# mosure/bevy_gaussian_splatting

Hardware: NVIDIA H100
Metric: rendered Msplats/sec @1080p, 6M-gaussian cloud (higher is better)
Workload: dtype f32 (f16-packed inputs)

## Files before the change

### bevy_gaussian_splatting_b200/csrc/project.cu

```cuda
#include <cuda_fp16.h>

#include "project_math.cuh"

namespace bgs {

__constant__ float c_shc[16] = {
    0.28209479177387814f, -0.4886025119029199f, 0.4886025119029199f, -0.4886025119029199f,
    1.0925484305920792f, -1.0925484305920792f, 0.31539156525252005f, -1.0925484305920792f,
    0.5462742152960396f, -0.5900435899266435f, 2.890611442640554f, -0.4570457994644658f,
    0.3731763325901154f, -0.4570457994644658f, 1.445305721320277f, -0.5900435899266435f};

__device__ __forceinline__ void normalize3(const float a[3], float out[3]) {
    const float inv = rsqrtf((a[0] * a[0] + a[1] * a[1]) + a[2] * a[2]);
    out[0] = a[0] * inv; out[1] = a[1] * inv; out[2] = a[2] * inv;
}
__device__ __forceinline__ float dot3(const float a[3], const float b[3]) {
    return (a[0] * b[0] + a[1] * b[1]) + a[2] * b[2];
}
__device__ __forceinline__ float srgb_to_linear(float v) {
    if (v <= 0.04045f) return v * (1.0f / 12.92f);
    return __powf((v + 0.055f) * (1.0f / 1.055f), 2.4f);
}
__device__ __forceinline__ uint32_t pack_bbox(float lo, float hi) {
    return (uint32_t)(int)lo | ((uint32_t)(int)hi << 16);
}
constexpr uint32_t BBOX_EMPTY = 1u;

__device__ __forceinline__ void make_bbox(float cx, float cy, float hx, float hy, int Wi, int Hi,
                                          uint32_t& bx, uint32_t& by) {
    bx = BBOX_EMPTY; by = BBOX_EMPTY;
    if (!(hx >= 0.0f) || !(hy >= 0.0f) || !(cx == cx) || !(cy == cy)) return;
    const float sx = hx * 1.0e-3f + 1.0e-2f, sy = hy * 1.0e-3f + 1.0e-2f;
    float x0 = ceilf((cx - hx) - (0.5f + sx));
    float x1 = floorf((cx + hx) - (0.5f - sx));
    float y0 = ceilf((cy - hy) - (0.5f + sy));
    float y1 = floorf((cy + hy) - (0.5f - sy));
    if (!(x0 <= x1) || !(y0 <= y1)) return;
    x0 = fmaxf(x0, 0.0f); y0 = fmaxf(y0, 0.0f);
    x1 = fminf(x1, (float)(Wi - 1)); y1 = fminf(y1, (float)(Hi - 1));
    if (!(x0 <= x1) || !(y0 <= y1)) return;
    bx = pack_bbox(x0, x1); by = pack_bbox(y0, y1);
}

template <bool F16>
struct Attr;
template <>
struct Attr<false> {
    __device__ static float4 load(const void* blocks, uint32_t id, float* sh, float q[4], float so[4], bool need_sh,
                                  uint32_t* = nullptr) {
        const float4* b = reinterpret_cast<const float4*>(blocks) + (size_t)id * 16;
        const float4 p = __ldg(b), r = __ldg(b + 1), s = __ldg(b + 2);
        q[0] = r.x; q[1] = r.y; q[2] = r.z; q[3] = r.w;
        so[0] = s.x; so[1] = s.y; so[2] = s.z; so[3] = s.w;
        if (need_sh) {
#pragma unroll
            for (int i = 0; i < 12; ++i) {
                const float4 v = __ldg(b + 3 + i);
                sh[4 * i] = v.x; sh[4 * i + 1] = v.y; sh[4 * i + 2] = v.z; sh[4 * i + 3] = v.w;
            }
        }
        return p;
    }
};
template <>
struct Attr<true> {
    __device__ static float lo(uint32_t w) { return __half2float(__ushort_as_half((unsigned short)(w & 0xFFFFu))); }
    __device__ static float hi(uint32_t w) { return __half2float(__ushort_as_half((unsigned short)(w >> 16))); }
    __device__ static float4 load(const void* blocks, uint32_t id, float* sh, float q[4], float so[4], bool need_sh,
                                  uint32_t* op_bits = nullptr) {
        const uint4* b = reinterpret_cast<const uint4*>(blocks) + (size_t)id * 8;
        const uint4 pw = __ldg(b), w = __ldg(b + 1);
        if (op_bits) *op_bits = w.w & 0xFFFFu;
        q[0] = hi(w.x); q[1] = lo(w.x); q[2] = hi(w.y); q[3] = lo(w.y);
        so[0] = hi(w.z); so[1] = lo(w.z); so[2] = hi(w.w); so[3] = lo(w.w);
        if (need_sh) {
#pragma unroll
            for (int i = 0; i < 6; ++i) {
                const uint4 v = __ldg(b + 2 + i);
                sh[8 * i] = lo(v.x); sh[8 * i + 1] = hi(v.x); sh[8 * i + 2] = lo(v.y); sh[8 * i + 3] = hi(v.y);
                sh[8 * i + 4] = lo(v.z); sh[8 * i + 5] = hi(v.z); sh[8 * i + 6] = lo(v.w); sh[8 * i + 7] = hi(v.w);
            }
        }
        return make_float4(__uint_as_float(pw.x), __uint_as_float(pw.y), __uint_as_float(pw.z), __uint_as_float(pw.w));
    }
};

template <bool F16>
__global__ void repack_kernel(const uint4* __restrict__ pos, const uint4* __restrict__ sh, const uint4* __restrict__ rot,
                              const uint4* __restrict__ so, uint32_t n, uint4* __restrict__ blocks) {
    constexpr uint32_t CH = F16 ? 8u : 16u;
    constexpr uint32_t SHC = F16 ? 6u : 12u;
    const size_t i = (size_t)blockIdx.x * blockDim.x + threadIdx.x;
    if (i >= (size_t)n * CH) return;
    const uint32_t id = (uint32_t)(i / CH), c = (uint32_t)(i % CH);
    uint4 v = make_uint4(0u, 0u, 0u, 0u);
    if (c == 0) v = pos[id];
    else if (c == 1) v = rot[id];
    else if (!F16 && c == 2) v = so[id];
    else {
        const uint32_t k = c - (F16 ? 2u : 3u);
        if (k < SHC) v = sh[(size_t)id * SHC + k];
    }
    blocks[i] = v;
}
void launch_repack(bool f16, const void* pos, const void* sh, const void* rot, const void* so, uint32_t n, void* blocks,
                   cudaStream_t stream) {
    const size_t total = (size_t)n * (f16 ? 8 : 16);
    const uint32_t grid = (uint32_t)((total + 255) / 256);
    if (f16) repack_kernel<true><<<grid, 256, 0, stream>>>((const uint4*)pos, (const uint4*)sh, (const uint4*)rot, (const uint4*)so, n, (uint4*)blocks);
    else repack_kernel<false><<<grid, 256, 0, stream>>>((const uint4*)pos, (const uint4*)sh, (const uint4*)rot, (const uint4*)so, n, (uint4*)blocks);
}

__global__ void depth_range_kernel(const float4* __restrict__ pos, uint32_t n, const uint32_t* __restrict__ sorted_payload,
                                   const uint32_t* __restrict__ slot_ids ,
                                   FrameCounters* __restrict__ ctr, FrameConsts fc) {
    if (threadIdx.x != 0 || blockIdx.x != 0 || n < 2u) return;
    const uint32_t n_vis = ctr->n_vis, n_sorted = ctr->n_sort;
    auto id_at = [&](uint32_t i) { const uint32_t p = sorted_payload[i]; return slot_ids ? slot_ids[p] : p; };
    uint32_t first, last;
    if (n_sorted == n) {
        first = id_at(1u); last = id_at(n - 1u);
    } else {
        const uint32_t cmin = 0xFFFFFFFFu - ctr->culled_min_inv, cmax = ctr->culled_max_p1 - 1u;
        first = n_vis >= 2u ? id_at(1u) : cmin;
        last = (n - n_vis) >= 1u ? cmax : id_at(n - 1u);
    }
    auto dist = [&](uint32_t id) {
        const float4 p = pos[id];
        float pw[4];
        mat4_point(fc.model, p.x, p.y, p.z, pw);
        const float d[3] = {pw[0] - fc.cam[0], pw[1] - fc.cam[1], pw[2] - fc.cam[2]};
        return sqrtf(dot3(d, d));
    };
    ctr->depth_min = dist(last);
    ctr->depth_max = dist(first);
}

__device__ __forceinline__ float adaptive_cutoff(float opacity) {
    const float a = 9.0f + 2.0f * det_ln(opacity);
    return sqrtf(a > 0.000001f ? a : 0.000001f);
}
__global__ void cutoff_table_kernel(float* __restrict__ tab) {
    const uint32_t h = blockIdx.x * blockDim.x + threadIdx.x;
    if (h < 65536u) tab[h] = adaptive_cutoff(__half2float(__ushort_as_half((unsigned short)h)));
}
void launch_cutoff_table(float* tab, cudaStream_t stream) { cutoff_table_kernel<<<256, 256, 0, stream>>>(tab); }

template <class ShLoader>
__device__ __forceinline__ void project_one(const FrameConsts& fc, const FrameCounters* __restrict__ ctr, uint32_t r, float4 p4,
                                            const float q[4], const float so[4], float cutoff_pre, ShLoader load_sh,
                                            SplatRec* __restrict__ recs, float4* __restrict__ extra, float4* __restrict__ aux) {
    SplatRec rec;
    rec.ux = 0.f; rec.uy = 0.f; rec.vx = 0.f; rec.vy = 0.f;
    rec.bx = BBOX_EMPTY; rec.by = BBOX_EMPTY;
    rec.r = 0.f; rec.g = 0.f; rec.b = 0.f;

    const KeyOut k = key_of(fc, p4.x, p4.y, p4.z);
    const float W = fc.W, H = fc.H;
    const float hw = 0.5f * W, hh = 0.5f * H;
    const float cx = k.ndc[0] * hw + hw;
    const float cy = hh - k.ndc[1] * hh;
    rec.cx = cx; rec.cy = cy;
    const float opacity = so[3];
    rec.op = opacity * fc.global_opacity;
    const bool drawn = k.visible && !(fc.draw_mode == BGS_DRAW_SELECTED && p4.w < 0.5f);

    float A[3][3];
#pragma unroll
    for (int rr = 0; rr < 3; ++rr)
#pragma unroll
        for (int cc = 0; cc < 3; ++cc) A[rr][cc] = fc.model[cc * 4 + rr];
    float Rm[3][3];
    {
        const float qr = q[0], x = q[1], y = q[2], z = q[3];
        Rm[0][0] = 1.0f - 2.0f * (y * y + z * z);
        Rm[1][0] = 2.0f * (x * y - qr * z);
        Rm[2][0] = 2.0f * (x * z + qr * y);
        Rm[0][1] = 2.0f * (x * y + qr * z);
        Rm[1][1] = 1.0f - 2.0f * (x * x + z * z);
        Rm[2][1] = 2.0f * (y * z - qr * x);
        Rm[0][2] = 2.0f * (x * z - qr * y);
        Rm[1][2] = 2.0f * (y * z + qr * x);
        Rm[2][2] = 1.0f - 2.0f * (x * x + y * y);
    }
    const float sc[3] = {so[0] * fc.global_scale, so[1] * fc.global_scale, so[2] * fc.global_scale};

    if (drawn) {
        float cutoff = 3.0f;
        if (fc.adaptive) {
            cutoff = cutoff_pre == cutoff_pre ? cutoff_pre : adaptive_cutoff(opacity);
        }
        if (fc.gaussian_mode == BGS_GAUSSIAN_3D) {
        float M[3][3], Sg[3][3], X[3][3], TS[3][3];
#pragma unroll
        for (int i = 0; i < 3; ++i)
#pragma unroll
            for (int j = 0; j < 3; ++j) M[i][j] = sc[i] * Rm[i][j];
#pragma unroll
        for (int i = 0; i < 3; ++i)
#pragma unroll
            for (int j = 0; j < 3; ++j) Sg[i][j] = (M[0][i] * M[0][j] + M[1][i] * M[1][j]) + M[2][i] * M[2][j];
        const float mn = fminf(fminf(fminf(fabsf(Sg[0][0]), fabsf(Sg[0][1])), fminf(fabsf(Sg[0][2]), fabsf(Sg[1][1]))),
                               fminf(fabsf(Sg[1][2]), fabsf(Sg[2][2])));
        const float mx = fmaxf(fmaxf(fmaxf(fabsf(Sg[0][0]), fabsf(Sg[0][1])), fmaxf(fabsf(Sg[0][2]), fabsf(Sg[1][1]))),
                               fmaxf(fabsf(Sg[1][2]), fabsf(Sg[2][2])));
        if (fc.model_identity && mn > 0.0f && mx < __uint_as_float(0x7F800000u) && Sg[0][0] == Sg[0][0] &&
            Sg[0][1] == Sg[0][1] && Sg[0][2] == Sg[0][2] && Sg[1][1] == Sg[1][1] && Sg[1][2] == Sg[1][2] && Sg[2][2] == Sg[2][2]) {
#pragma unroll
            for (int i = 0; i < 3; ++i)
#pragma unroll
                for (int j = 0; j < 3; ++j) TS[i][j] = Sg[i][j];
        } else {
#pragma unroll
        for (int i = 0; i < 3; ++i)
#pragma unroll
            for (int j = 0; j < 3; ++j) X[i][j] = (A[i][0] * Sg[0][j] + A[i][1] * Sg[1][j]) + A[i][2] * Sg[2][j];
#pragma unroll
        for (int i = 0; i < 3; ++i)
#pragma unroll
            for (int j = 0; j < 3; ++j) TS[i][j] = (X[i][0] * A[j][0] + X[i][1] * A[j][1]) + X[i][2] * A[j][2];
        }
        float c3[6] = {TS[0][0], TS[1][0], TS[2][0], TS[1][1], TS[2][1], TS[2][2]};
        if (fc.cov_pre) {
            c3[0] = q[0]; c3[1] = q[1]; c3[2] = q[2]; c3[3] = q[3]; c3[4] = so[0]; c3[5] = so[1];
        }
        const float Vrk[3][3] = {{c3[0], c3[1], c3[2]}, {c3[1], c3[3], c3[4]}, {c3[2], c3[4], c3[5]}};
        float tv[4];
        mat4_point(fc.view_from_world, k.pw[0], k.pw[1], k.pw[2], tv);
        const float fx = fc.p00 * W, fy = fc.p11 * H;
        const float sz = 1.0f / (tv[2] * tv[2]);
        const float J00 = fx / tv[2], J20 = -(fx * tv[0]) * sz;
        const float J11 = -fy / tv[2], J21 = (fy * tv[1]) * sz;
        float Tm[3][2];
#pragma unroll
        for (int i = 0; i < 3; ++i) {
            const float v0 = fc.view_from_world[i * 4 + 0], v1 = fc.view_from_world[i * 4 + 1],
                        v2 = fc.view_from_world[i * 4 + 2];
            Tm[i][0] = v0 * J00 + v2 * J20;
            Tm[i][1] = v1 * J11 + v2 * J21;
        }
        float Y[3][2];
#pragma unroll
        for (int i = 0; i < 3; ++i)
#pragma unroll
            for (int b = 0; b < 2; ++b) Y[i][b] = (Vrk[i][0] * Tm[0][b] + Vrk[i][1] * Tm[1][b]) + Vrk[i][2] * Tm[2][b];
        const float a = ((Tm[0][0] * Y[0][0] + Tm[1][0] * Y[1][0]) + Tm[2][0] * Y[2][0]) + 0.3f;
        const float b = (Tm[0][1] * Y[0][0] + Tm[1][1] * Y[1][0]) + Tm[2][1] * Y[2][0];
        const float c = ((Tm[0][1] * Y[0][1] + Tm[1][1] * Y[1][1]) + Tm[2][1] * Y[2][1]) + 0.3f;
        const float det = a * c - b * b;
        const float mid = 0.5f * (a + c);
        const float disc = fmaxf(0.0f, mid * mid - det);
        const float term = sqrtf(disc);
        const float l1 = mid + term;
        if (fc.aabb) {
            const float l2 = fmaxf(mid - term, 0.0f);
            const float Rq = cutoff * fmaxf(sqrtf(l1), sqrtf(l2));
            const float dinv = 1.0f / det;
            rec.ux = c * dinv; rec.uy = -b * dinv; rec.vx = a * dinv; rec.vy = Rq;
            const float h = 0.5f * Rq;
            make_bbox(cx, cy, h, h, fc.Wi, fc.Hi, rec.bx, rec.by);
        } else {
        const float aa = (a - c) * (a - c);
        const float bb = sqrtf(aa + (4.0f * b) * b);
        const float major = sqrtf(((a + c) + bb) * 0.5f);
        const float minor = sqrtf(((a + c) - bb) * 0.5f);
        const float Bx = cutoff * major, By = cutoff * minor;
        const float evx = -b, evy = l1 - a;
        const float el = sqrtf(evx * evx + evy * evy);
        const float e1x = evx / el, e1y = evy / el;
        const float e2x = e1y, e2y = -e1x;
        rec.ux = (2.0f * e1x) / Bx; rec.uy = (-2.0f * e1y) / Bx;
        rec.vx = (2.0f * e2x) / By; rec.vy = (-2.0f * e2y) / By;
        const float hx = 0.5f * (fabsf(e1x) * Bx + fabsf(e2x) * By);
        const float hy = 0.5f * (fabsf(e1y) * Bx + fabsf(e2y) * By);
        if (rec.ux == rec.ux && rec.uy == rec.uy && rec.vx == rec.vx && rec.vy == rec.vy)
            make_bbox(cx, cy, hx, hy, fc.Wi, fc.Hi, rec.bx, rec.by);
        }
        } else {
            float L[3][2];
#pragma unroll
            for (int j = 0; j < 2; ++j) {
                const float rc[3] = {Rm[j][0] * sc[j], Rm[j][1] * sc[j], Rm[j][2] * sc[j]};
#pragma unroll
                for (int i = 0; i < 3; ++i) L[i][j] = (A[i][0] * rc[0] + A[i][1] * rc[1]) + A[i][2] * rc[2];
            }
            float G[3][4];
            mat4_dir(fc.clip_from_world, L[0][0], L[1][0], L[2][0], G[0]);
            mat4_dir(fc.clip_from_world, L[0][1], L[1][1], L[2][1], G[1]);
            mat4_point(fc.clip_from_world, k.pw[0], k.pw[1], k.pw[2], G[2]);
            const float fxk = fc.p00 * W / 2.0f, fyk = fc.p11 * H / 2.0f;
            const float cxk = (W - 1.0f) / 2.0f, cyk = (H - 1.0f) / 2.0f;
            float T0[3], T1[3], T2[3];
#pragma unroll
            for (int j = 0; j < 3; ++j) {
                T0[j] = fxk * G[j][0] + cxk * G[j][3];
                T1[j] = fyk * G[j][1] + cyk * G[j][3];
                T2[j] = G[j][3];
            }
            const float c2 = cutoff * cutoff;
            const float test[3] = {c2, c2, -1.0f};
            const float tt[3] = {test[0] * T2[0], test[1] * T2[1], test[2] * T2[2]};
            const float d = dot3(tt, T2);
            float Rq = 0.0f, mean0 = 0.0f, mean1 = 0.0f;
            bool ok = !(fabsf(d) < 1.0e-4f);
            if (ok) {
                const float inv = 1.0f / d;
                const float f[3] = {inv * test[0], inv * test[1], inv * test[2]};
                const float t02[3] = {T0[0] * T2[0], T0[1] * T2[1], T0[2] * T2[2]};
                const float t12[3] = {T1[0] * T2[0], T1[1] * T2[1], T1[2] * T2[2]};
                mean0 = dot3(f, t02); mean1 = dot3(f, t12);
                const float f0[3] = {f[0] * T0[0], f[1] * T0[1], f[2] * T0[2]};
                const float f1[3] = {f[0] * T1[0], f[1] * T1[1], f[2] * T1[2]};
                const float ex = mean0 * mean0 - dot3(f0, T0);
                const float ey = mean1 * mean1 - dot3(f1, T1);
                if (ex < 1.0e-4f || ey < 1.0e-4f) ok = false;
                else Rq = fmaxf(fmaxf(sqrtf(ex), sqrtf(ey)), cutoff * 0.707106f);
            }
            if (ok) {
                rec.ux = 2.0f / Rq; rec.uy = 0.0f; rec.vx = 0.0f; rec.vy = -2.0f / Rq;
                const float h = 0.5f * Rq;
                if (Rq == Rq) make_bbox(cx, cy, h, h, fc.Wi, fc.Hi, rec.bx, rec.by);
                if (fc.aabb && extra != nullptr) {
                    float4* e = extra + (size_t)r * 4;
                    e[0] = make_float4(Rq, mean0, mean1, W / H);
                    e[1] = make_float4(T0[0], T0[1], T0[2], 0.0f);
                    e[2] = make_float4(T1[0], T1[1], T1[2], 0.0f);
                    e[3] = make_float4(T2[0], T2[1], T2[2], 0.0f);
                }
            }
        }

        float rgb[3] = {0.f, 0.f, 0.f};
        if (fc.rasterize_mode == BGS_RASTERIZE_COLOR) {
            float sh[48];
            load_sh(sh);
            const float dlt[3] = {k.pw[0] - fc.cam[0], k.pw[1] - fc.cam[1], k.pw[2] - fc.cam[2]};
            float dw[3], loc[3], dl[3];
            normalize3(dlt, dw);
            if (fc.model_identity) {
                loc[0] = dw[0]; loc[1] = dw[1]; loc[2] = dw[2];
            } else {
#pragma unroll
                for (int cc = 0; cc < 3; ++cc) {
                    const float col[3] = {A[0][cc], A[1][cc], A[2][cc]};
                    float bn[3];
                    normalize3(col, bn);
                    loc[cc] = dot3(bn, dw);
                }
            }
            normalize3(loc, dl);
            const float x = dl[0], y = dl[1], z = dl[2];
            const float xx = x * x, yy = y * y, zz = z * z;
            float basis[16];
            basis[0] = 1.0f;
            basis[1] = y; basis[2] = z; basis[3] = x;
            basis[4] = x * y; basis[5] = y * z; basis[6] = (2.0f * zz - xx) - yy;
            basis[7] = x * z; basis[8] = xx - yy;
            basis[9] = y * (3.0f * xx - yy);
            basis[10] = (x * y) * z;
            basis[11] = y * ((4.0f * zz - xx) - yy);
            basis[12] = z * ((2.0f * zz - 3.0f * xx) - 3.0f * yy);
            basis[13] = x * ((4.0f * zz - xx) - yy);
            basis[14] = z * (xx - yy);
            basis[15] = x * (xx - 3.0f * yy);
#pragma unroll
            for (int kk = 0; kk < 16; ++kk) basis[kk] *= c_shc[kk];
#pragma unroll
            for (int cc = 0; cc < 3; ++cc) {
                float acc = 0.5f;
#pragma unroll
                for (int kk = 0; kk < 16; ++kk) acc = fmaf(sh[3 * kk + cc], basis[kk], acc);
                rgb[cc] = acc;
            }
            if (fc.color_space == 0u) {
#pragma unroll
                for (int cc = 0; cc < 3; ++cc) rgb[cc] = srgb_to_linear(rgb[cc]);
            }
        }
        float drgb[3] = {0.f, 0.f, 0.f}, nrgb[3] = {0.f, 0.f, 0.f};
        if (fc.rasterize_mode == BGS_RASTERIZE_DEPTH || fc.aux) {
            float* rgb = drgb;
            const float dlt[3] = {k.pw[0] - fc.cam[0], k.pw[1] - fc.cam[1], k.pw[2] - fc.cam[2]};
            const float depth = sqrtf(dot3(dlt, dlt));
            const float dmin = ctr->depth_min, dmax = ctr->depth_max;
            if (fc.n_cloud >= 2u) {
            float nd = (depth - dmin) / (dmax - dmin);
            nd = fminf(fmaxf(nd, 0.0f), 1.0f);
            float t1 = (nd - 0.5f) / (1.0f - 0.5f); t1 = fminf(fmaxf(t1, 0.0f), 1.0f);
            float t2 = (nd - 0.0f) / (0.5f - 0.0f); t2 = fminf(fmaxf(t2, 0.0f), 1.0f);
            rgb[0] = t1 * t1 * (3.0f - 2.0f * t1);
            rgb[1] = 1.0f - fabsf(nd - 0.5f) * 2.0f;
            rgb[2] = 1.0f - t2 * t2 * (3.0f - 2.0f * t2);
            }
        }
        if (fc.rasterize_mode == BGS_RASTERIZE_POSITION) {
#pragma unroll
            for (int cc = 0; cc < 3; ++cc) rgb[cc] = (k.pw[cc] - fc.aabb_min[cc]) / (fc.aabb_max[cc] - fc.aabb_min[cc]);
        }
        if (fc.rasterize_mode == BGS_RASTERIZE_NORMAL || fc.aux) {
            float* rgb = nrgb;
            float SR[3], Ln[3], wn[4];
#pragma unroll
            for (int i = 0; i < 3; ++i) SR[i] = sc[i] * Rm[i][2];
#pragma unroll
            for (int i = 0; i < 3; ++i) Ln[i] = (A[i][0] * SR[0] + A[i][1] * SR[1]) + A[i][2] * SR[2];
            mat4_dir(fc.view_from_world, Ln[0], Ln[1], Ln[2], wn);
            const float l = sqrtf(((wn[0] * wn[0] + wn[1] * wn[1]) + wn[2] * wn[2]) + wn[3] * wn[3]);
#pragma unroll
            for (int cc = 0; cc < 3; ++cc) rgb[cc] = 0.5f * (wn[cc] / l + 1.0f);
        }
        if (fc.rasterize_mode == BGS_RASTERIZE_DEPTH) { rgb[0] = drgb[0]; rgb[1] = drgb[1]; rgb[2] = drgb[2]; }
        if (fc.rasterize_mode == BGS_RASTERIZE_NORMAL) { rgb[0] = nrgb[0]; rgb[1] = nrgb[1]; rgb[2] = nrgb[2]; }
        rec.r = rgb[0]; rec.g = rgb[1]; rec.b = rgb[2];
        if (fc.draw_mode == BGS_DRAW_HIGHLIGHT_SELECTED && p4.w > 0.5f) {
            rec.r = 0.3f; rec.g = 1.0f; rec.b = 0.1f; rec.op = 1.0f;
            drgb[0] = nrgb[0] = 0.3f; drgb[1] = nrgb[1] = 1.0f; drgb[2] = nrgb[2] = 0.1f;
        }
        if (fc.aux && aux != nullptr) {
            aux[(size_t)r * 2] = make_float4(drgb[0], drgb[1], drgb[2], 0.0f);
            aux[(size_t)r * 2 + 1] = make_float4(nrgb[0], nrgb[1], nrgb[2], 0.0f);
        }
    }
    float4* out = reinterpret_cast<float4*>(recs + r);
    out[0] = make_float4(rec.cx, rec.cy, rec.ux, rec.uy);
    out[1] = make_float4(rec.vx, rec.vy, __uint_as_float(rec.bx), __uint_as_float(rec.by));
    out[2] = make_float4(rec.r, rec.g, rec.b, rec.op);
}

constexpr int PROJ_MIN_CTAS = 6;
template <bool F16>
__global__ void __launch_bounds__(128, PROJ_MIN_CTAS)
project_kernel(const void* __restrict__ blocks, const uint32_t* __restrict__ index_list, int by_slot,
               const FrameCounters* __restrict__ ctr, FrameConsts fc, SplatRec* __restrict__ recs,
               float4* __restrict__ extra , const float* __restrict__ cutoff_tab,
               float4* __restrict__ aux ) {
    const uint32_t n_vis = ctr->n_vis;
    for (uint32_t r = blockIdx.x * blockDim.x + threadIdx.x; r < n_vis; r += gridDim.x * blockDim.x) {
        const uint32_t id = by_slot ? __ldg(index_list + r) : __ldg(index_list + (n_vis - 1u - r));
        float sh[48], q[4], so[4];
        const bool need_sh = fc.rasterize_mode == BGS_RASTERIZE_COLOR;
        uint32_t op_bits = 0u;
        const float4 p4 = Attr<F16>::load(blocks, id, sh, q, so, need_sh, &op_bits);
        const float cutoff_pre = (F16 && fc.adaptive) ? __ldg(cutoff_tab + op_bits) : __uint_as_float(0x7FC00000u);
        project_one(fc, ctr, r, p4, q, so, cutoff_pre,
                    [&](float* out) {
#pragma unroll
                        for (int i = 0; i < 48; ++i) out[i] = sh[i];
                    },
                    recs, extra, aux);
    }
}

void launch_depth_range(const float4* pos, uint32_t n, const uint32_t* sorted_payload, const uint32_t* slot_ids,
                        FrameCounters* ctr, const FrameConsts& fc, cudaStream_t stream) {
    depth_range_kernel<<<1, 32, 0, stream>>>(pos, n, sorted_payload, slot_ids, ctr, fc);
}

void launch_project(bool f16, const void* blocks, const uint32_t* index_list, int by_slot, const FrameCounters* ctr,
                    const FrameConsts& fc, SplatRec* recs, float4* extra, uint32_t n_hint, int sm_count,
                    const float* cutoff_tab, float4* aux, cudaStream_t stream) {
    uint32_t grid = (n_hint + 127) / 128;
    if (grid > 65535u * 8u) grid = 65535u * 8u;
    if (grid < (uint32_t)sm_count) grid = (uint32_t)sm_count;
    if (f16) project_kernel<true><<<grid, 128, 0, stream>>>(blocks, index_list, by_slot, ctr, fc, recs, extra, cutoff_tab, aux);
    else project_kernel<false><<<grid, 128, 0, stream>>>(blocks, index_list, by_slot, ctr, fc, recs, extra, cutoff_tab, aux);
}

}
```

Measured before the change: 16520.

## Stage gathered splat blocks into shared memory with warp-cooperative cp.async

Replaces each thread's own gather of its splat's attribute block with a warp-cooperative copy. Lanes are shuffled splat ids so each cp.async instruction fetches contiguous chunks of a few splats, written into a per-warp, XOR-swizzled shared-memory stage. Threads then decode position, rotation/scale and SH from shared memory, and the next batch's index lookup is prefetched. Each CTA now walks multiple batches, the grid is sized for two batches per CTA, and the min-CTAs launch bound is raised. The cost is extra shared memory, warp syncs and a single-buffered wait with little real overlap between copy and compute.

```diff
diff --git a/bevy_gaussian_splatting_b200/csrc/project.cu b/bevy_gaussian_splatting_b200/csrc/project.cu
--- a/bevy_gaussian_splatting_b200/csrc/project.cu
+++ b/bevy_gaussian_splatting_b200/csrc/project.cu
@@ -43,47 +43,70 @@
 }
 
 template <bool F16>
-struct Attr;
+struct BlockLayout {
+    static constexpr uint32_t CH = F16 ? 8u : 16u;
+    static constexpr uint32_t GEO = F16 ? 2u : 3u;
+    static constexpr uint32_t END = F16 ? 8u : 15u;
+};
+template <bool F16>
+struct Staged;
 template <>
-struct Attr<false> {
-    __device__ static float4 load(const void* blocks, uint32_t id, float* sh, float q[4], float so[4], bool need_sh,
-                                  uint32_t* = nullptr) {
-        const float4* b = reinterpret_cast<const float4*>(blocks) + (size_t)id * 16;
-        const float4 p = __ldg(b), r = __ldg(b + 1), s = __ldg(b + 2);
+struct Staged<false> {
+    const uint4* row;
+    uint32_t sw;
+    __device__ float4 chunk(uint32_t c) const {
+        const uint4 v = row[c ^ sw];
+        return make_float4(__uint_as_float(v.x), __uint_as_float(v.y), __uint_as_float(v.z), __uint_as_float(v.w));
+    }
+    __device__ float4 pos() const { return chunk(0); }
+    __device__ uint32_t op_bits() const { return 0u; }
+    __device__ void attrs(float q[4], float so[4]) const {
+        const float4 r = chunk(1), s = chunk(2);
         q[0] = r.x; q[1] = r.y; q[2] = r.z; q[3] = r.w;
         so[0] = s.x; so[1] = s.y; so[2] = s.z; so[3] = s.w;
-        if (need_sh) {
-#pragma unroll
-            for (int i = 0; i < 12; ++i) {
-                const float4 v = __ldg(b + 3 + i);
-                sh[4 * i] = v.x; sh[4 * i + 1] = v.y; sh[4 * i + 2] = v.z; sh[4 * i + 3] = v.w;
-            }
-        }
-        return p;
+    }
+    __device__ void sh(float* sh) const {
+#pragma unroll
+        for (int i = 0; i < 12; ++i) {
+            const float4 v = chunk(3 + i);
+            sh[4 * i] = v.x; sh[4 * i + 1] = v.y; sh[4 * i + 2] = v.z; sh[4 * i + 3] = v.w;
+        }
     }
 };
 template <>
-struct Attr<true> {
+struct Staged<true> {
+    const uint4* row;
+    uint32_t sw;
     __device__ static float lo(uint32_t w) { return __half2float(__ushort_as_half((unsigned short)(w & 0xFFFFu))); }
     __device__ static float hi(uint32_t w) { return __half2float(__ushort_as_half((unsigned short)(w >> 16))); }
-    __device__ static float4 load(const void* blocks, uint32_t id, float* sh, float q[4], float so[4], bool need_sh,
-                                  uint32_t* op_bits = nullptr) {
-        const uint4* b = reinterpret_cast<const uint4*>(blocks) + (size_t)id * 8;
-        const uint4 pw = __ldg(b), w = __ldg(b + 1);
-        if (op_bits) *op_bits = w.w & 0xFFFFu;
+    __device__ uint4 chunk(uint32_t c) const { return row[c ^ sw]; }
+    __device__ float4 pos() const {
+        const uint4 pw = chunk(0);
+        return make_float4(__uint_as_float(pw.x), __uint_as_float(pw.y), __uint_as_float(pw.z), __uint_as_float(pw.w));
+    }
+    __device__ uint32_t op_bits() const { return row[1u ^ sw].w & 0xFFFFu; }
+    __device__ void attrs(float q[4], float so[4]) const {
+        const uint4 w = chunk(1);
         q[0] = hi(w.x); q[1] = lo(w.x); q[2] = hi(w.y); q[3] = lo(w.y);
         so[0] = hi(w.z); so[1] = lo(w.z); so[2] = hi(w.w); so[3] = lo(w.w);
-        if (need_sh) {
-#pragma unroll
-            for (int i = 0; i < 6; ++i) {
-                const uint4 v = __ldg(b + 2 + i);
-                sh[8 * i] = lo(v.x); sh[8 * i + 1] = hi(v.x); sh[8 * i + 2] = lo(v.y); sh[8 * i + 3] = hi(v.y);
-                sh[8 * i + 4] = lo(v.z); sh[8 * i + 5] = hi(v.z); sh[8 * i + 6] = lo(v.w); sh[8 * i + 7] = hi(v.w);
-            }
-        }
-        return make_float4(__uint_as_float(pw.x), __uint_as_float(pw.y), __uint_as_float(pw.z), __uint_as_float(pw.w));
+    }
+    __device__ void sh(float* sh) const {
+#pragma unroll
+        for (int i = 0; i < 6; ++i) {
+            const uint4 v = chunk(2 + i);
+            sh[8 * i] = lo(v.x); sh[8 * i + 1] = hi(v.x); sh[8 * i + 2] = lo(v.y); sh[8 * i + 3] = hi(v.y);
+            sh[8 * i + 4] = lo(v.z); sh[8 * i + 5] = hi(v.z); sh[8 * i + 6] = lo(v.w); sh[8 * i + 7] = hi(v.w);
+        }
     }
 };
+
+__device__ __forceinline__ void cp_async16(void* smem, const void* gmem) {
+    asm volatile("cp.async.cg.shared.global [%0], [%1], 16;\n" ::"r"((uint32_t)__cvta_generic_to_shared(smem)), "l"(gmem)
+                 : "memory");
+}
+__device__ __forceinline__ void cp_async_commit() { asm volatile("cp.async.commit_group;\n" ::: "memory"); }
+template <int N>
+__device__ __forceinline__ void cp_async_wait() { asm volatile("cp.async.wait_group %0;\n" ::"n"(N) : "memory"); }
 
 template <bool F16>
 __global__ void repack_kernel(const uint4* __restrict__ pos, const uint4* __restrict__ sh, const uint4* __restrict__ rot,
@@ -427,27 +450,66 @@
     out[2] = make_float4(rec.r, rec.g, rec.b, rec.op);
 }
 
-constexpr int PROJ_MIN_CTAS = 6;
+constexpr int PROJ_THREADS = 128;
+constexpr int PROJ_WARPS = PROJ_THREADS / 32;
+constexpr int PROJ_MIN_CTAS = 7;
+constexpr uint32_t PROJ_BATCHES = 2;
 template <bool F16>
-__global__ void __launch_bounds__(128, PROJ_MIN_CTAS)
+constexpr size_t proj_smem_bytes() { return (size_t)PROJ_WARPS * 32u * (F16 ? 8u : 16u) * 16u; }
+
+template <bool F16>
+__global__ void __launch_bounds__(PROJ_THREADS, PROJ_MIN_CTAS)
 project_kernel(const void* __restrict__ blocks, const uint32_t* __restrict__ index_list, int by_slot,
                const FrameCounters* __restrict__ ctr, FrameConsts fc, SplatRec* __restrict__ recs,
                float4* __restrict__ extra , const float* __restrict__ cutoff_tab,
                float4* __restrict__ aux ) {
+    using L = BlockLayout<F16>;
+    constexpr uint32_t PER_INSN = 32u / L::CH;
+    constexpr uint32_t NONE = 0xFFFFFFFFu;
+    extern __shared__ __align__(16) uint4 s_stage[];
+    const uint32_t lane = threadIdx.x & 31u;
+    uint4* const stage = s_stage + (size_t)(threadIdx.x >> 5) * 32u * L::CH;
     const uint32_t n_vis = ctr->n_vis;
-    for (uint32_t r = blockIdx.x * blockDim.x + threadIdx.x; r < n_vis; r += gridDim.x * blockDim.x) {
-        const uint32_t id = by_slot ? __ldg(index_list + r) : __ldg(index_list + (n_vis - 1u - r));
-        float sh[48], q[4], so[4];
-        const bool need_sh = fc.rasterize_mode == BGS_RASTERIZE_COLOR;
-        uint32_t op_bits = 0u;
-        const float4 p4 = Attr<F16>::load(blocks, id, sh, q, so, need_sh, &op_bits);
-        const float cutoff_pre = (F16 && fc.adaptive) ? __ldg(cutoff_tab + op_bits) : __uint_as_float(0x7FC00000u);
-        project_one(fc, ctr, r, p4, q, so, cutoff_pre,
-                    [&](float* out) {
-#pragma unroll
-                        for (int i = 0; i < 48; ++i) out[i] = sh[i];
-                    },
-                    recs, extra, aux);
+    const uint32_t n_chunks = fc.rasterize_mode == BGS_RASTERIZE_COLOR ? L::END : L::GEO;
+    const uint32_t stride = gridDim.x * (uint32_t)PROJ_THREADS;
+    auto id_of = [&](uint32_t base) -> uint32_t {
+        const uint32_t r = base + lane;
+        if (base >= n_vis || r >= n_vis) return NONE;
+        return by_slot ? __ldg(index_list + r) : __ldg(index_list + (n_vis - 1u - r));
+    };
+    auto copy_batch = [&](uint32_t id) {
+        const uint32_t c = lane % L::CH;
+#pragma unroll
+        for (uint32_t i = 0; i < L::CH; ++i) {
+            const uint32_t j = i * PER_INSN + lane / L::CH;
+            const uint32_t idj = __shfl_sync(0xFFFFFFFFu, id, j);
+            if (idj != NONE && c < n_chunks)
+                cp_async16(stage + j * L::CH + (c ^ (j & 7u)), static_cast<const uint4*>(blocks) + (size_t)idj * L::CH + c);
+        }
+        cp_async_commit();
+    };
+
+    uint32_t base = blockIdx.x * (uint32_t)PROJ_THREADS + (threadIdx.x & ~31u);
+    if (base >= n_vis) return;
+    copy_batch(id_of(base));
+    uint32_t id_next = id_of(base + stride);
+    for (;;) {
+        const uint32_t next = base + stride;
+        cp_async_wait<0>();
+        __syncwarp();
+        const uint32_t r = base + lane;
+        if (r < n_vis) {
+            const Staged<F16> blk{stage + lane * L::CH, lane & 7u};
+            const float cutoff_pre = (F16 && fc.adaptive) ? __ldg(cutoff_tab + blk.op_bits()) : __uint_as_float(0x7FC00000u);
+            float q[4], so[4];
+            blk.attrs(q, so);
+            project_one(fc, ctr, r, blk.pos(), q, so, cutoff_pre, [&](float* out) { blk.sh(out); }, recs, extra, aux);
+        }
+        __syncwarp();
+        if (next >= n_vis) break;
+        copy_batch(id_next);
+        id_next = id_of(next + stride);
+        base = next;
     }
 }
 
@@ -459,11 +521,16 @@
 void launch_project(bool f16, const void* blocks, const uint32_t* index_list, int by_slot, const FrameCounters* ctr,
                     const FrameConsts& fc, SplatRec* recs, float4* extra, uint32_t n_hint, int sm_count,
                     const float* cutoff_tab, float4* aux, cudaStream_t stream) {
-    uint32_t grid = (n_hint + 127) / 128;
+    const uint32_t per_cta = (uint32_t)PROJ_THREADS * PROJ_BATCHES;
+    uint32_t grid = (n_hint + per_cta - 1) / per_cta;
     if (grid > 65535u * 8u) grid = 65535u * 8u;
     if (grid < (uint32_t)sm_count) grid = (uint32_t)sm_count;
-    if (f16) project_kernel<true><<<grid, 128, 0, stream>>>(blocks, index_list, by_slot, ctr, fc, recs, extra, cutoff_tab, aux);
-    else project_kernel<false><<<grid, 128, 0, stream>>>(blocks, index_list, by_slot, ctr, fc, recs, extra, cutoff_tab, aux);
-}
-
-}
+    if (f16)
+        project_kernel<true><<<grid, PROJ_THREADS, proj_smem_bytes<true>(), stream>>>(blocks, index_list, by_slot, ctr, fc, recs,
+                                                                                      extra, cutoff_tab, aux);
+    else
+        project_kernel<false><<<grid, PROJ_THREADS, proj_smem_bytes<false>(), stream>>>(blocks, index_list, by_slot, ctr, fc, recs,
+                                                                                        extra, cutoff_tab, aux);
+}
+
+}
```

Measured after the change: 17300 (median of 6 runs). 1.05x the previous value.
